# IntuitionMachines/volta

Measured on AMD Instinct MI355X. Metric: image-text pairs/sec, ctrl_vilbert_base pretrain step, higher is better.
Workload: dtype bf16

## Files before the change

include/volta_hip.h:

```cpp
#ifndef VOLTA_HIP_H
#define VOLTA_HIP_H
#include <stddef.h>
#include <stdint.h>

#ifdef __cplusplus
extern "C" {
#endif

typedef void* vk_stream_t;

int vk_version(void);
const char* vk_device_arch(void);
const char* vk_last_error(void);

typedef struct vk_dropout {
    const uint64_t* seed;
    uint32_t site;
    uint32_t threshold;
    float scale;
} vk_dropout;

int vk_set_seed(uint64_t* seed_dev, uint64_t seed, vk_stream_t s);

int vk_cast_f32_bf16(const float* src, void* dst, int64_t n, vk_stream_t s);
// ... 242 lines not shown
    const float* target;
    const int64_t* labels;
    const float* conf;
    const int32_t* pos;
    const int32_t* count;
    const int32_t* neg_index;
    float* lse;
    float* aux;
    float* loss_sum;
    float weight;
    int32_t V, ld, max_rows, kind, n_neg;
} vk_vis_loss_args;
int vk_vis_loss_fwd(const vk_vis_loss_args* a, vk_stream_t s);
int vk_vis_loss_bwd(const vk_vis_loss_args* a, void* dlogits, int ldd, const float* gscale, vk_stream_t s);
int vk_nce_negatives(vk_dropout rng, int B, int R, int32_t* out, vk_stream_t s);

enum { VK_TASK_BCE_SCALED = 0, VK_TASK_BCE_MEAN = 1, VK_TASK_BCE_REGIONS = 2, VK_TASK_CE_OPTIONS = 3 };
typedef struct vk_task_loss_args {
    const float* logits;
    const void* target;
    const int64_t* mask;
    void* work;
    float* out;
    int32_t* row_argmax;
    int32_t kind, groups, n, ld;
} vk_task_loss_args;
int64_t vk_task_loss_work_bytes(int groups);
int vk_task_loss_fwd(const vk_task_loss_args* a, vk_stream_t s);
int vk_task_loss_bwd(const vk_task_loss_args* a, const float* gscale, void* dlogits, vk_stream_t s);

int vk_mask_prep(const int64_t* mask, float* out, int n, vk_stream_t s);

#define VK_CHUNK_SKIP 255
int vk_grad_norm_workspace_floats(void);
int vk_grad_norm_clip(const float* g, int64_t n, float pre_scale, float max_norm, float* partial, float* out, vk_stream_t s);
int vk_grad_norm_clip_masked(const float* g, int64_t n, const uint8_t* chunk_class, float pre_scale, float max_norm, float* partial, float* out, vk_stream_t s);
int vk_grad_sqnorm_chunks(const float* g, int64_t chunk0, int64_t nchunks, const uint8_t* chunk_class, float* sums, vk_stream_t s);
int vk_grad_norm_from_chunks(float* sums, int64_t total_chunks, float pre_scale, float max_norm, float* out, vk_stream_t s);
typedef struct vk_adamw_args {
    float* p;
    const float* g;
    float* m;
    float* v;
    void* shadow;
    const uint8_t* chunk_class;
    const float* clip;
    int64_t n;
    float cls_lr_mult[8];
    float cls_wd[8];
    float lr, beta1, beta2, eps, step_mult, grad_scale;
} vk_adamw_args;
int vk_adamw_step(const vk_adamw_args* a, vk_stream_t s);
int vk_adamw_step_on(const vk_adamw_args* a, int ncus, vk_stream_t s);
typedef struct vk_adamw_tensor {
    float* p;
    const float* g;
    float* m;
    float* v;
    int64_t numel;
    int32_t cls;
    int32_t reserved_;
} vk_adamw_tensor;
int vk_adamw_step_list(const vk_adamw_args* a, const vk_adamw_tensor* list, int n, int64_t max_numel, vk_stream_t s);
int vk_grad_sqnorm_list(const vk_adamw_tensor* list, int n, int64_t max_numel, float* work, float* sums, vk_stream_t s);
int vk_grad_sqnorm_list_work_floats(void);
#define VK_RADAM_CLASSES 64
// ... 7 lines not shown
    const float* clip;
    int64_t n;
    float cls_decay[VK_RADAM_CLASSES];
    float cls_step[VK_RADAM_CLASSES];
    int32_t cls_rect[VK_RADAM_CLASSES];
    float beta1, beta2;
    float one_minus_beta1, one_minus_beta2;
    float eps, grad_scale;
} vk_radam_args;
int vk_radam_step(const vk_radam_args* a, vk_stream_t s);
int vk_radam_step_list(const vk_radam_args* a, const vk_adamw_tensor* list, int n, int64_t max_numel, vk_stream_t s);
int vk_axpy_f32(float* y, const float* x, float alpha, int64_t n, vk_stream_t s);
int vk_sum_slabs_f32(float* dst, const float* src, int64_t slab_stride, int nslabs, int64_t n, vk_stream_t s);
int vk_sum_slabs_bf16(void* dst, const float* src, int64_t slab_stride, int nslabs, int64_t n, const int32_t* dyn_rows, int row_len, vk_stream_t s);
int vk_memset_async(void* p, int value, int64_t bytes, vk_stream_t s);
int vk_hold_cus(int nwg, int usec, int whole_cu, vk_stream_t s);
int vk_gate_wait(const uint64_t* flag, const uint64_t* stamp, int timeout_us, int32_t* err, vk_stream_t s);
int vk_bump_u64(uint64_t* word, vk_stream_t s);
int vk_store_u64(uint64_t* word, uint64_t value, vk_stream_t s);
int vk_gate_value(const uint64_t* flag, uint64_t want, int timeout_us, int32_t* err, vk_stream_t s);
int vk_comm_standin(const void* src, void* dst, int64_t bytes, int nwg, int min_usec, uint64_t* stamps, vk_stream_t s);
int vk_gemm_reserve_cus(int n);
#define VK_TAIL_MAX_JOBS 16
typedef struct vk_tail_job {
    float* dst;
    float* dst2;
    const float* src;
    const float* src2;
    int64_t stride;
    int64_t n;
    int32_t kind, count;
    int32_t accumulate;
    int32_t block_start;
} vk_tail_job;
int vk_side_tail(const vk_tail_job* jobs, int njobs, vk_stream_t s);

int vk_mul_bf16(const void* a, const void* b, void* out, int64_t n, const int32_t* dyn_rows, int row_len, vk_stream_t s);

enum {
    VK_OP_GEMM = 1,
    VK_OP_LN_FWD, VK_OP_LN_BWD,
    VK_OP_ATTN_FWD,
    VK_OP_ATTN_BWD,
    VK_OP_EMBED_FWD, VK_OP_EMBED_BWD, VK_OP_XENT_FWD,
    VK_OP_XENT_BWD,
    VK_OP_KL_FWD, VK_OP_KL_BWD,
    VK_OP_GENERIC,
    VK_OP_SIDE_BEGIN, VK_OP_SIDE_END, VK_OP_WAIT_SIDE, VK_OP_JOIN,
    VK_OP_LN_FINALIZE,
    VK_OP_GEMM_FP8,
    VK_OP_GEMM_CHAIN
};
enum {
    VK_FN_CAST = 1, VK_FN_MEMSET, VK_FN_LOC_FWD, VK_FN_LOC_BWD, VK_FN_ADD_DROPOUT, VK_FN_COLSUM, VK_FN_SELECT,
    VK_FN_GATHER, VK_FN_SCATTER_ADD, VK_FN_LOSS_FINAL, VK_FN_POOL_FWD, VK_FN_POOL_BWD, VK_FN_MASK_PREP, VK_FN_MUL,
    VK_FN_VLBERT_PREP, VK_FN_VLBERT_MASKGRAD, VK_FN_ROWGROUP_SUM, VK_FN_RELU_BWD, VK_FN_COPY, VK_FN_SUM_SLABS, VK_FN_SUM_SLABS_BF16,
    VK_FN_SIDE_TAIL,
    VK_FN_QUANT_ROWS,
    VK_FN_CAST_FP8,
    VK_FN_VIS_LOSS_FWD,
    VK_FN_VIS_LOSS_BWD,
    VK_FN_NCE_NEG,
    VK_FN_TEXT_END_ROWS,
    VK_FN_VLBERT_OBJ_IDS,
    VK_FN_VLBERT_POSITIONS,
    VK_FN_HOLD,
// ... 129 lines not shown
```

volta_amd/_lib.py:

```python
import ctypes as C
import os

import torch

_HERE = os.path.dirname(os.path.abspath(__file__))
LIB_PATH = os.path.join(_HERE, "libvolta_hip_%s.so" % os.environ["VK_LIB"] if os.environ.get("VK_LIB") else "libvolta_hip.so")
GEMM_PERSISTENT, GEMM_ONE_TILE_PER_WG, GEMM_SOFT_START = 0x1000, 0x2000, 0x4000


class VoltaHipError(RuntimeError):
    pass


if not os.path.exists(LIB_PATH):
    raise ImportError(
        "volta_amd: %s not found. The HIP kernels are the product; there is no fallback path. "
        "Build with `make -C volta_amd/csrc` (hipcc --offload-arch=gfx950)." % LIB_PATH)

lib = C.CDLL(LIB_PATH)

c_p = C.c_void_p
i32 = C.c_int32
CHUNK_SKIP = 255


class Dropout(C.Structure):
    _fields_ = [("seed", c_p), ("site", C.c_uint32), ("threshold", C.c_uint32), ("scale", C.c_float)]


def dropout_cfg(seed_ptr, site, p):
    if p <= 0.0 or not seed_ptr:
        return Dropout(None, 0, 0, 1.0)
    return Dropout(seed_ptr, site, min(int(p * 4294967296.0), 0xFFFFFFFF), 1.0 / (1.0 - p))


def rng_cfg(seed_ptr, site):
    return Dropout(seed_ptr, site, 0, 1.0)


class GemmProblem(C.Structure):
    _fields_ = [("A", c_p), ("B", c_p), ("C", c_p), ("C2", c_p), ("bias", c_p), ("R", c_p), ("bias_grad", c_p),
                ("dyn", c_p), ("M", i32), ("N", i32), ("K", i32), ("lda", i32), ("ldb", i32), ("ldc", i32),
                ("ldr", i32), ("n_store", i32), ("ws", c_p), ("cnt", c_p), ("part", i32), ("nparts", i32),
                ("sig", c_p), ("dep", c_p), ("err", c_p), ("dep_need", i32), ("reserved_", i32), ("retire_flag", c_p), ("retire_stamp", c_p)]


class GemmFp8Problem(C.Structure):
    _fields_ = [("p", GemmProblem), ("scale_a", c_p), ("scale_b", c_p), ("c8", c_p), ("c8_mul", C.c_float), ("ldc8", i32)]


GEMM_FP8_MAX_GROUP = 4


class DropRows(C.Structure):
    _fields_ = [("site", C.c_uint32), ("div", i32), ("mul", i32), ("off", i32)]

# ... 85 lines not shown


class GradSeedArgs(C.Structure):
    _fields_ = [("src", c_p), ("stride_b", C.c_int64), ("stride_l", C.c_int64), ("dst", c_p), ("y", c_p), ("B", i32), ("L", i32), ("H", i32),
                ("row0", i32), ("ld", i32), ("ldy", i32), ("accumulate", i32), ("reserved_", i32)]


PAIR_MAX_SEGS = 8


class PairGatherArgs(C.Structure):
    _fields_ = [("src", c_p * PAIR_MAX_SEGS), ("dst", c_p * PAIR_MAX_SEGS), ("bytes", C.c_int64 * PAIR_MAX_SEGS), ("side", i32 * PAIR_MAX_SEGS),
                ("cap_idx", c_p), ("img_idx", c_p), ("n_items", C.c_int64 * 2), ("nseg", i32), ("npairs", i32), ("c0", i32), ("nc", i32),
                ("i0", i32), ("ni", i32)]


TASK_MAX_SEGS, TASK_ROWS = 2, 4
TASK_TARGET_NONE, TASK_TARGET_SCATTER, TASK_TARGET_IOU = range(3)


class TaskBatchArgs(C.Structure):
    _fields_ = [(n, c_p) for n in ("feat", "boxes", "n", "wh", "mean", "segs", "mask_count", "features", "spatials", "image_mask", "target", "csr",
                                   "labels", "scores", "ref_box")] + \
               [(n, i32) for n in ("S", "Rcap", "F", "N", "R", "B", "num_locs", "add_global", "target_kind", "num_labels")]


class TaskImage(C.Structure):
    _fields_ = [("feat_b64", c_p), ("feat_len", C.c_size_t), ("boxes_b64", c_p), ("boxes_len", C.c_size_t), ("feat", c_p), ("boxes", c_p),
                ("rows", i32), ("F", i32)]


class TailJob(C.Structure):
    _fields_ = [("dst", c_p), ("dst2", c_p), ("src", c_p), ("src2", c_p), ("stride", C.c_int64), ("n", C.c_int64), ("kind", i32), ("count", i32),
                ("accumulate", i32), ("block_start", i32)]


TAIL_MAX_JOBS = 16


class GenericArgs(C.Structure):
    _fields_ = [("fn", i32), ("p", c_p * 6), ("n", C.c_int64 * 6), ("f", C.c_float * 2), ("drop", Dropout)]


class Op(C.Structure):
    _fields_ = [("kind", i32), ("i0", i32), ("i1", i32), ("i2", i32), ("a", c_p), ("b", c_p), ("c", c_p)]


(OP_GEMM, OP_LN_FWD, OP_LN_BWD, OP_ATTN_FWD, OP_ATTN_BWD, OP_EMBED_FWD, OP_EMBED_BWD, OP_XENT_FWD, OP_XENT_BWD,
 OP_KL_FWD, OP_KL_BWD, OP_GENERIC, OP_SIDE_BEGIN, OP_SIDE_END, OP_WAIT_SIDE, OP_JOIN, OP_LN_FINALIZE, OP_GEMM_FP8, OP_GEMM_CHAIN) = range(1, 20)
(FN_CAST, FN_MEMSET, FN_LOC_FWD, FN_LOC_BWD, FN_ADD_DROPOUT, FN_COLSUM, FN_SELECT, FN_GATHER, FN_SCATTER_ADD,
 FN_LOSS_FINAL, FN_POOL_FWD, FN_POOL_BWD, FN_MASK_PREP, FN_MUL, FN_VLBERT_PREP, FN_VLBERT_MASKGRAD, FN_ROWGROUP_SUM,
 FN_RELU_BWD, FN_COPY, FN_SUM_SLABS, FN_SUM_SLABS_BF16, FN_SIDE_TAIL, FN_QUANT_ROWS, FN_CAST_FP8, FN_VIS_LOSS_FWD, FN_VIS_LOSS_BWD,
 FN_NCE_NEG, FN_TEXT_END_ROWS, FN_VLBERT_OBJ_IDS, FN_VLBERT_POSITIONS, FN_HOLD, FN_GATE, FN_BUMP, FN_GRAD_SEED) = range(1, 35)


class AttnArgs(C.Structure):
    _fields_ = [("q", c_p * 2), ("k", c_p * 2), ("v", c_p * 2), ("ld", i32 * 2), ("L", i32 * 2), ("mask", c_p * 2),
                ("ctx", c_p * 2), ("ldo", i32 * 2), ("lse", c_p * 2), ("B", i32), ("nh", i32), ("gate", (i32 * 2) * 2),
                ("drop", (Dropout * 2) * 2), ("scale", C.c_float), ("dh", i32), ("probs", (c_p * 2) * 2)]


class AttnBwdArgs(C.Structure):
    _fields_ = [("dctx", c_p * 2), ("dq", c_p * 2), ("dk", c_p * 2), ("dv", c_p * 2), ("ldg", i32 * 2)]


NT, NN, TN = 0, 1, 2
EPI_BF16, EPI_GELU, EPI_MULR, EPI_ADDR, EPI_F32, EPI_RELU, EPI_F32_ACC = range(7)
# ... 143 lines not shown
```

volta_amd/csrc/optim.hip:

```cpp
#include "common.h"
#include "../../include/volta_hip.h"
#include "util.h"

namespace vk {

constexpr int NORM_BLOCKS = 1024;

__global__ __launch_bounds__(256) void sqnorm_partial_kernel(const float* g, size_t n4, float* partial, const uint8_t* chunk_class) {
    __shared__ float sh[4];
    float s = 0.f;
    for (size_t i = (size_t)blockIdx.x * 256 + threadIdx.x; i < n4; i += (size_t)gridDim.x * 256) {
        if (chunk_class && chunk_class[i >> 8] == VK_CHUNK_SKIP) continue;
        const f32x4 v = *(const f32x4*)(g + i * 4);
        s += v[0] * v[0] + v[1] * v[1] + v[2] * v[2] + v[3] * v[3];
    }
    s = wave_sum(s);
    if ((threadIdx.x & 63) == 0) sh[threadIdx.x >> 6] = s;
    __syncthreads();
    if (threadIdx.x == 0) partial[blockIdx.x] = sh[0] + sh[1] + sh[2] + sh[3];
}
__global__ __launch_bounds__(256) void sqnorm_final_kernel(const float* partial, int nblk, float pre_scale, float max_norm, float* out) {
    __shared__ double sh[4];
    double s = 0.0;
    for (int i = threadIdx.x; i < nblk; i += 256) s += (double)partial[i];
    for (int o = 32; o > 0; o >>= 1) s += __shfl_xor(s, o, 64);
    if ((threadIdx.x & 63) == 0) sh[threadIdx.x >> 6] = s;
    __syncthreads();
    if (threadIdx.x == 0) {
        const float norm = (float)sqrt(sh[0] + sh[1] + sh[2] + sh[3]) * pre_scale;
        out[0] = norm;
        float coef = 1.f;
        if (max_norm > 0.f) { coef = max_norm / (norm + 1e-6f); if (coef > 1.f) coef = 1.f; }
        out[1] = coef;
    }
}

__global__ __launch_bounds__(256) void sqnorm_chunks_kernel(const float* g, size_t chunk0, size_t nchunks, const uint8_t* chunk_class, float* sums) {
    const size_t c = (size_t)blockIdx.x * 4 + (threadIdx.x >> 6);
    if (c >= nchunks) return;
    const size_t chunk = chunk0 + c;
    const int lane = threadIdx.x & 63;
    float s = 0.f;
    if (!(chunk_class && chunk_class[chunk] == VK_CHUNK_SKIP)) {
        const float* p = g + chunk * 1024;
#pragma unroll
        for (int k = 0; k < 4; ++k) {
            const f32x4 v = __builtin_nontemporal_load((const f32x4*)(p + (k * 64 + lane) * 4));
            s += v[0] * v[0] + v[1] * v[1] + v[2] * v[2] + v[3] * v[3];
        }
    }
    s = wave_sum(s);
    if (lane == 0) sums[chunk] = s;
}
constexpr int SQ_GROUPS = 128;
__global__ __launch_bounds__(256) void sqnorm_groups_kernel(const float* sums, size_t n, double* group) {
    __shared__ double sh[4];
    const size_t per = (n + SQ_GROUPS - 1) / SQ_GROUPS, lo = (size_t)blockIdx.x * per, hi = lo + per < n ? lo + per : n;
    double s = 0.0;
    for (size_t i = lo + threadIdx.x; i < hi; i += 256) s += (double)sums[i];
    for (int o = 32; o > 0; o >>= 1) s += __shfl_xor(s, o, 64);
    if ((threadIdx.x & 63) == 0) sh[threadIdx.x >> 6] = s;
    __syncthreads();
    if (threadIdx.x == 0) group[blockIdx.x] = (sh[0] + sh[1]) + (sh[2] + sh[3]);
}
__global__ __launch_bounds__(64) void sqnorm_from_groups_kernel(const double* group, float pre_scale, float max_norm, float* out) {
    double s = group[threadIdx.x] + group[threadIdx.x + 64];
    for (int o = 32; o > 0; o >>= 1) s += __shfl_xor(s, o, 64);
    if (threadIdx.x == 0) {
        const float norm = (float)sqrt(s) * pre_scale;
        out[0] = norm;
        float coef = 1.f;
        if (max_norm > 0.f) { coef = max_norm / (norm + 1e-6f); if (coef > 1.f) coef = 1.f; }
        out[1] = coef;
    }
}

__device__ __forceinline__ void adamw_element(float& p, float& m, float& v, float g, float gs, float b1, float b2, float eps, float step, float lr_wd) {
#pragma clang fp contract(off)
    const float gr = g * gs;
    m = __builtin_fmaf(b1, m, (1.f - b1) * gr);
    v = __builtin_fmaf(b2, v, ((1.f - b2) * gr) * gr);
    p = __builtin_fmaf(-step, m / (sqrtf(v) + eps), p);
    if (lr_wd > 0.f) p = __builtin_fmaf(-lr_wd, p, p);
}
// ... 142 lines not shown
        float a = 0.f;
        for (int s = 0; s < nslabs; ++s) a += src[(size_t)s * stride + i];
        dst[i] = a;
    }
}

__global__ __launch_bounds__(256) void sum_slabs_bf16_kernel(uint16_t* dst, const float* src, size_t stride, int nslabs, size_t n, const int32_t* dyn_rows, int row_len) {
    if (dyn_rows) { const size_t lim = (size_t)(*dyn_rows) * row_len; if (lim < n) n = lim; }
    const size_t n4 = n >> 2;
    for (size_t i = (size_t)blockIdx.x * 256 + threadIdx.x; i < n4; i += (size_t)gridDim.x * 256) {
        f32x4 a = *(const f32x4*)(src + i * 4);
        for (int s = 1; s < nslabs; ++s) {
            const f32x4 b = *(const f32x4*)(src + (size_t)s * stride + i * 4);
#pragma unroll
            for (int r = 0; r < 4; ++r) a[r] += b[r];
        }
        *(u32x2*)(dst + i * 4) = u32x2{pack2bf(a[0], a[1]), pack2bf(a[2], a[3])};
    }
}

struct TailJobs { vk_tail_job j[VK_TAIL_MAX_JOBS]; int32_t njobs; };

__global__ __launch_bounds__(256) void side_tail_kernel(const TailJobs t) {
    __shared__ float red[16][17];
    int ji = 0;
#pragma unroll
    for (int i = 1; i < VK_TAIL_MAX_JOBS; ++i)
        if (i < t.njobs && (int)blockIdx.x >= t.j[i].block_start) ji = i;
    const vk_tail_job& J = t.j[ji];
    const int blk = (int)blockIdx.x - J.block_start;
    if (J.kind == 0) {
        const size_t n4 = (size_t)J.n >> 2;
        const size_t i = (size_t)blk * 256 + threadIdx.x;
        if (i < n4) {
            f32x4 a = __builtin_nontemporal_load((const f32x4*)(J.src + i * 4));
            for (int s = 1; s < J.count; ++s) {
                const f32x4 b = __builtin_nontemporal_load((const f32x4*)(J.src + (size_t)s * J.stride + i * 4));
#pragma unroll
                for (int r = 0; r < 4; ++r) a[r] += b[r];
            }
            __builtin_nontemporal_store(a, (f32x4*)(J.dst + i * 4));
        }
        if (blk == 0 && threadIdx.x < (J.n & 3)) {
            const size_t k = n4 * 4 + threadIdx.x;
            float a = 0.f;
            for (int s = 0; s < J.count; ++s) a += J.src[(size_t)s * J.stride + k];
            J.dst[k] = a;
        }
    } else {
        const int H = (int)J.n, tx = threadIdx.x & 15, ty = threadIdx.x >> 4;
        const int i = blk * 16 + tx;
        float s = 0.f;
        if (i < 2 * H) {
            for (int b = ty; b < J.count; b += 16) s += J.src[(size_t)b * 2 * H + i];
            if (J.src2)
                for (int b = ty; b < (int)J.stride; b += 16) s += J.src2[(size_t)b * 2 * H + i];
        }
        red[ty][tx] = s;
        __syncthreads();
        if (ty == 0 && i < 2 * H) {
#pragma unroll
            for (int k = 1; k < 16; ++k) s += red[k][tx];
            float* o = i < H ? J.dst + i : J.dst2 + (i - H);
            *o = J.accumulate ? *o + s : s;
        }
    }
}

}

using namespace vk;

extern "C" int vk_side_tail(const vk_tail_job* jobs, int njobs, vk_stream_t s) {
    if (njobs <= 0) return 0;
    if (njobs > VK_TAIL_MAX_JOBS) return set_error("vk_side_tail: %d jobs (max %d)", njobs, VK_TAIL_MAX_JOBS);
    TailJobs t;
    t.njobs = njobs;
    int total = 0;
    for (int i = 0; i < njobs; ++i) {
        t.j[i] = jobs[i];
        vk_tail_job& J = t.j[i];
        int nb;
        if (J.kind == 0) {
            if ((J.stride & 3) || ((uintptr_t)J.dst & 15) || ((uintptr_t)J.src & 15)) return set_error("vk_side_tail: slab job %d needs 16-byte alignment", i);
            nb = (int)((J.n / 4 + 255) / 256);
            if (nb < 1) nb = 1;
        } else if (J.kind == 1) {
            nb = (int)((2 * J.n + 15) / 16);
        } else return set_error("vk_side_tail: unknown job kind %d", J.kind);
        if (J.n <= 0 || J.count <= 0) nb = 0;
        J.block_start = total;
        total += nb;
    }
    if (total == 0) return 0;
    hipLaunchKernelGGL(side_tail_kernel, dim3((unsigned)total), dim3(256), 0, (hipStream_t)s, t);
    return check_launch("vk_side_tail");
}

extern "C" int vk_sum_slabs_bf16(void* dst, const float* src, int64_t slab_stride, int nslabs, int64_t n, const int32_t* dyn_rows, int row_len, vk_stream_t s) {
    if (n <= 0 || nslabs <= 0) return 0;
    if ((slab_stride & 3) || (n & 3) || (row_len & 3)) return set_error("vk_sum_slabs_bf16: lengths must be multiples of 4");
    if (((uintptr_t)src & 15) || ((uintptr_t)dst & 7)) return set_error("vk_sum_slabs_bf16: src needs 16-byte, dst 8-byte alignment");
    int64_t blocks = (n / 4 + 255) / 256;
    if (blocks > 2048) blocks = 2048;
    hipLaunchKernelGGL(sum_slabs_bf16_kernel, dim3((unsigned)blocks), dim3(256), 0, (hipStream_t)s, (uint16_t*)dst, src, (size_t)slab_stride, nslabs, (size_t)n, dyn_rows, row_len);
    return check_launch("vk_sum_slabs_bf16");
}

extern "C" int vk_sum_slabs_f32(float* dst, const float* src, int64_t slab_stride, int nslabs, int64_t n, vk_stream_t s) {
    if (n <= 0 || nslabs <= 0) return 0;
    if ((slab_stride & 3) || ((uintptr_t)dst & 15) || ((uintptr_t)src & 15)) return set_error("vk_sum_slabs_f32: 16-byte alignment required");
    int64_t blocks = (n / 4 + 255) / 256;
    if (blocks > 2048) blocks = 2048;
    if (blocks < 1) blocks = 1;
    hipLaunchKernelGGL(sum_slabs_kernel, dim3((unsigned)blocks), dim3(256), 0, (hipStream_t)s, dst, src, (size_t)slab_stride, nslabs, (size_t)n);
    return check_launch("vk_sum_slabs_f32");
}

extern "C" int vk_grad_norm_workspace_floats(void) { return NORM_BLOCKS; }

extern "C" int vk_grad_norm_clip_masked(const float* g, int64_t n, const uint8_t* chunk_class, float pre_scale, float max_norm, float* partial, float* out, vk_stream_t s) {
// ... 83 lines not shown
```

volta_amd/engine.py:

```python
import ctypes as C
import math
import os

import torch

from . import _lib as L
from ._lib import check, ptr
from .modules import sublayer_schedule

CHUNK = 1024
VIS_TARGET_WIDTH = {"0": 1601, "1": 2048, "2": 2048, "3": 1600, "4": 400, "5": 2048, "6": 1601}
NO_DECAY = ("bias", "LayerNorm.bias", "LayerNorm.weight")


def _round_up(x, m):
    return (x + m - 1) // m * m


class ParamArena:

    def __init__(self, model, device, prefix=""):
        named = [(prefix + n, p) for n, p in model.named_parameters()]
        byname = dict(named)
        slots, seen = [], set()
# ... 13 lines not shown
        self.offset, self.shape = {}, {}
        classes = []
        off = 0
        for group in slots:
            start = off
            for g in group:
                self.offset[g] = off
                self.shape[g] = tuple(byname[g].shape)
                off += byname[g].numel()
            off = _round_up(off, CHUNK)
            nd = any(k in group[0] for k in NO_DECAY)
            assert all(any(k in g for k in NO_DECAY) == nd for g in group)
            classes += [1 if nd else 0] * ((off - start) // CHUNK)
        self.total = off
        self.device = device
        self.master = torch.zeros(self.total, dtype=torch.float32, device=device)
        self.shadow = torch.zeros(self.total, dtype=torch.bfloat16, device=device)
        self.grad = torch.zeros(self.total, dtype=torch.float32, device=device)
        self.chunk_class = torch.tensor(classes, dtype=torch.uint8, device=device)
        self.names = [n for n, _ in named]
        self.params = byname
        with torch.no_grad():
            for name, p in named:
                v = self.view(name)
                v.copy_(p.data.to(device=device, dtype=torch.float32))
                p.data = v
                p.grad = None
        self.shadow_version = -1
        self.weights_epoch = 0
        self.fp8_sites = {}
        self.fp8_epoch = -1
        self._plist = self._gviews = None
        self.opt_pending = None

    def view(self, name, which="master"):
        buf = getattr(self, which)
        o = self.offset[name]
        n = 1
        for d in self.shape[name]:
            n *= d
        return buf[o:o + n].view(self.shape[name])

    def param_list(self):
        if self._plist is None or len(self._plist) != len(self.params):
            self._plist = list(self.params.items())
        return self._plist

    def grad_views(self):
        if self._gviews is None or len(self._gviews) != len(self.params):
            self._gviews = [self.view(n, "grad") for n in self.params]
        return self._gviews

    def span(self, names, which, shape):
        buf = getattr(self, which)
        o = self.offset[names[0]]
        n = 1
        for d in shape:
            n *= d
        for a, b in zip(names[:-1], names[1:]):
            assert self.offset[b] == self.offset[a] + int(torch.tensor(self.shape[a]).prod())
        return buf[o:o + n].view(shape)

    def intact(self):
        return all(p.data_ptr() == self.master.data_ptr() + 4 * self.offset[n] for n, p in self.params.items())

    def param_version(self):
        return sum(p._version for p in self.params.values()) + self.master._version

    def refresh_shadow(self, force=False):
        v = self.param_version()
        if force or self.shadow_version != v:
            self.sync_optimizer()
            check(L.lib.vk_cast_f32_bf16(ptr(self.master), ptr(self.shadow), self.total, L.stream_ptr()))
            self.shadow_version = v
            self.weights_epoch += 1

    def mark_shadow_fresh(self):
        self.shadow_version = self.param_version()
        self.weights_epoch += 1

    def fp8_weight(self, w):
        key = w.data_ptr()
        if key not in self.fp8_sites:
            N, K = w.shape
            Kp = _round_up(K, 128)
            self.fp8_sites[key] = (w, torch.zeros(N, Kp, dtype=torch.uint8, device=self.device), torch.ones(N, dtype=torch.float32, device=self.device))
            self.fp8_epoch = -1
        return self.fp8_sites[key][1:]

    def refresh_fp8(self):
        if self.fp8_epoch == self.weights_epoch:
            return
        for w, q, sc in self.fp8_sites.values():
            N, K = w.shape
# ... 105 lines not shown
        if self.wide and fp8:
            raise NotImplementedError("the fp8 projection path covers the single-width (ctrl_*) geometry")
        if self.wide and cfg.image_embeddings != "vilbert":
            raise NotImplementedError("different stream widths are built for the ViLBERT embeddings (config/vilbert_base.json)")
        if cfg.hidden_act != "gelu" or cfg.v_hidden_act != "gelu":
            raise NotImplementedError("engine supports gelu activations (every reference config)")
        if cfg.fusion_method not in ("mul", "sum", "text", "vl-bert_vqa", "none"):
            raise ValueError("Invalid fusion method: %s" % cfg.fusion_method)
        self.unused_params = set()
        if T + Rv > 512:
            raise NotImplementedError("more than 512 keys per query row (%d text + %d vision rows)" % (T, Rv))
        self.H, self.I, self.nh = H, cfg.intermediate_size, cfg.num_attention_heads
        self.st = [Stream(T, B, H), Stream(Rv, B, Hv)]
        self.R = Rv - (1 if cfg.add_global_imgfeat is not None else 0)
        self.bufs = {}
        self.keep = []
        self.fwd, self.bwd = Plan(), Plan()
        self.bwd_groups = []
        self.site = 0
        self.seed = torch.zeros(1, dtype=torch.int64, device=dev)
        self.inputs = {}
        self.taps = {}
        self.grad_seeds = {}
        self.losses = None
        self.nce_site = None
        self.task_loss_bufs = None
        self._aside = ""
        self._split_cur = {}
        self._soft_zero_b_listed = False
        self._n_ln_partial = 0
        self._deferred_ln = []
        self._n_gate, self._gate_flag = 0, None
        self._slab_cursor = 0
        self._fwd_segments = {}
        self._build()

    def buf(self, name, shape, dtype=torch.bfloat16, zero=False):
        assert name not in self.bufs, name
        t = (torch.zeros if zero else torch.empty)(shape, dtype=dtype, device=self.dev)
        self.bufs[name] = t
        return t

    def embed_ws(self, eb, tag):
        n = L.lib.vk_embed_bwd_workspace_bytes(eb.M, eb.H, eb.V, eb.P, int(bool(eb.pos_ids) and bool(eb.dpos)))
        eb.work = _addr(self.tmp("embed_ws_" + tag, (max(n, 1),), torch.uint8))
        return eb

    def tmp(self, name, shape, dtype=torch.bfloat16):
        name += self._aside
        if name not in self.bufs:
            self.bufs[name] = torch.empty(shape, dtype=dtype, device=self.dev)
        t = self.bufs[name]
        assert tuple(t.shape) == tuple(shape) and t.dtype == dtype, (name, t.shape, shape)
        return t

    def drop(self, p):
        site = self.site
        self.site += 1
        return L.dropout_cfg(self.seed.data_ptr(), site, p if self.train else 0.0)

    def k(self, obj):
        self.keep.append(obj)
        return obj

    def patch(self, name, struct, field, index=None):
        self.inputs.setdefault(name, []).append((struct, field, index))
# ... 216 lines not shown
        self.sublayer_ids = [n for n, _ in sched]
        backbone = self.heads == "backbone"
        v_level0 = []
        for k, (n, typ) in enumerate(sched):
            self.sub_k = k
            self.fwd_sub_start.append(len(self.fwd.ops))
            if emb_image_aside and k == k_vis:
                f.append((L.OP_WAIT_SIDE, 15, 0, 0, None, None, None))
            ops = self._attn_sublayer(n) if typ == "attn" else self._ffn_sublayer(n)
            if k + 2 < self.n_sub:
                ops.insert(0, (L.OP_WAIT_SIDE, (k + 2) % 8, 0, 0, None, None, None))
            if backbone and k + 1 < self.n_sub:
                head = []
                for m, tag in ((0, "t"), (1, "v")):
                    op = self._seed_op("%s%d" % (tag, n), self._dx(m, self.level[m] % 2), self.B, self.st[m].L, self.st[m].H, accumulate=1)
                    (v_level0 if (m == 1 and emb_image_aside and self.level[1] == 0) else head).append(op)
                ops[0:0] = head
            if emb_image_aside and k == k_vis:
                ops = ops + v_level0 + emb_image_bwd
            bwd_stages.append(ops)
            self.taps["t%d" % n], self.taps["v%d" % n] = self.x[0], self.x[1]
        self.fwd_heads_start = len(self.fwd.ops)
        head_bwd = self._heads() if self.heads == "pretrain" else self._heads_tasks()
        self.bwd.ops = list(self.bwd_pro) + list(head_bwd)
        self.bwd_marks = [len(self.bwd.ops)]
        for ops in reversed(bwd_stages):
            self.bwd.ops += ops
            self.bwd_marks.append(len(self.bwd.ops))
        self.bwd.ops.append((L.OP_JOIN, 0, 0, 0, None, None, None))
        prefixes = [["bert.t_pooler.", "bert.v_pooler.", "cls.", "clfs_dict."]] + [pf for pf in reversed(self.stage_prefix)]
        self.param_ready_stage = {}
        for name in self.arena.params:
            self.param_ready_stage[name] = max(i for i, pf in enumerate(prefixes) if any(name.startswith(q) for q in pf))
        self.fwd.freeze()
        self.bwd.freeze()

    def _build_score(self):
        cfg, B, T, Rv = self.cfg, self.B, self.T, self.Rv
        f = self.fwd.ops
        text_subs, vision_subs, per_modality = self.split
        kinds = dict(sublayer_schedule(cfg))
        self.x, self.x8, self.level, self.bwd_pro = [None, None], [None, None], [0, 0], []
        self.masks = [self.buf("mask_t", (B, T), torch.float32), self.buf("mask_v", (B, Rv), torch.float32)]
        kind = cfg.image_embeddings

        def mask_prep(m, src=None):
            g = self.generic(L.FN_MASK_PREP, p=(src, self.masks[m]), n=(B * self.st[m].L,))
            if src is None:
                self.patch(("attention_mask", "image_attention_mask")[m], g, "p", 0)
            f.append((L.OP_GENERIC, 0, 0, 0, g, None, None))

        def sublayers(ns):
            for n in ns:
                self._attn_sublayer(n) if kinds[n] == "attn" else self._ffn_sublayer(n)

        if self.part in ("text", "image"):
            m = 0 if self.part == "text" else 1
            subs = text_subs if m == 0 else vision_subs
            if not per_modality:
                raise ValueError("image_embeddings=%r mixes the modalities in its embedding: there is no per-modality prefix" % kind)
            if subs:
                mask_prep(m)
            if m == 0:
                self._emb_text("bert.embeddings.")
            elif kind == "uniter":
                self._emb_image_uniter("bert.embeddings.")
# ... 649 lines not shown
            du[m] = self.tmp("du%d_%d%s" % (m, par, wtag), (self.st[m].M, Im[m]))
        self._ln_pair(b, L.OP_LN_BWD, lnb)
        d1 = [self.prob(dd[m], self.W(names[m]["down"] + ".weight"), du[m], self.st[m].M, Im[m], Hm[m], Hm[m], Im[m], Im[m], R=gp[m], ldr=Im[m]) for m in ms]
        d2 = [self.prob(du[m], self.W(names[m]["up"] + ".weight"), dxn[m], self.st[m].M, Hm[m], Im[m], Im[m], Hm[m], Hm[m], R=dz[m], ldr=Hm[m]) for m in ms]
        chained = self.chain == "all" and not self.fp8 and self._soft_pair_ok([(self.st[m].M, Im[m], Hm[m]) for m in ms])
        if chained:
            for m, p1, p2 in zip(ms, d1, d2):
                p1.sig, p1.err = self.soft_counters(self.st[m].M // 256, backward=True)
                p2.dep, p2.err, p2.dep_need = p1.sig, p1.err, Im[m] // 256
            self.gemm_chain(b, L.NN, L.EPI_MULR, d1, L.EPI_ADDR, d2)
        else:
            self.gemm(b, L.NN, L.EPI_MULR, d1)
        gate_mode, self.side_gate = self.side_gate, self.side_gate and not chained
        self._wgrad(b, ms, shared, [lambda m: (dd[m], h[m], self.G(names[m]["down"] + ".weight"), self.G(names[m]["down"] + ".bias"), Hm[m], Im[m], Hm[m], Im[m]),
                                    lambda m: (du[m], x_in[m], self.G(names[m]["up"] + ".weight"), self.G(names[m]["up"] + ".bias"), Im[m], Hm[m], Im[m], Hm[m])])
        self.side_gate = gate_mode
        if not chained:
            self.gemm(b, L.NN, L.EPI_ADDR, self.retire_on(d2))
        return b

    def _wgrad(self, b, ms, shared, specs):
        jobs = []
        for spec in specs:
            per_w = {}
            for m in ms:
                dY, X, gW, gB, Mo, No, lda, ldb = spec(m)
                key = gW.data_ptr()
                per_w.setdefault(key, (gW, gB, Mo, No, []))[4].append((dY, X, self.st[m].M, lda, ldb))
            jobs += list(per_w.values())
        chunk_rows = 5120.0
        tiles = lambda cr: sum(-(-Mo // 256) * -(-No // 256) * sum(max(1, int(round(rows / cr))) for _, _, rows, _, _ in srcs) for _, _, Mo, No, srcs in jobs)
        while chunk_rows > 1280 and tiles(chunk_rows) < 130:
            chunk_rows /= 2
        probs, reduces = [], []
        for gW, gB, Mo, No, srcs in jobs:
            chunks = []
            for dY, X, rows, lda, ldb in srcs:
                ns = max(1, int(round(rows / chunk_rows)))
                step = -(-rows // ns)
                step = -(-step // 64) * 64
                r0 = 0
                while r0 < rows:
                    chunks.append((dY[r0:], X[r0:], min(step, rows - r0), lda, ldb))
                    r0 += step
            if len(chunks) == 1:
                dY, X, rows, lda, ldb = chunks[0]
                probs.append(self.prob(dY, X, gW, Mo, No, rows, lda, ldb, No, bias_grad=gB))
                continue
            stride = _round_up(Mo * No + Mo, 4)
            slab = self._slab(len(chunks) * stride)
            for i, (dY, X, rows, lda, ldb) in enumerate(chunks):
                base = slab[i * stride:]
                probs.append(self.prob(dY, X, base, Mo, No, rows, lda, ldb, No, bias_grad=base[Mo * No:]))
            reduces.append((gW, slab, stride, len(chunks), Mo * No))
            reduces.append((gB, slab[Mo * No:], stride, len(chunks), Mo))
        assert len(probs) <= 32, "too many wgrad problems in one group"
        gate = self._gate_words() if self.side_gate else None
        b.append((L.OP_SIDE_BEGIN, 1 if gate is not None else 0, 0, 0, None, None, None))
        if gate is not None:
            self._n_gate += 1
            assert self._n_gate < gate.numel()
            flag = gate.data_ptr() + 8 * self._n_gate
            b.append((L.OP_GENERIC, 0, 0, 0, self.generic(L.FN_GATE, p=(flag, gate.data_ptr(), self.bufs["gate_err"]), n=(1000000,)), None, None))
            self._gate_flag = (flag, gate.data_ptr())
        if self.side_delay_us > 0:
            b.append((L.OP_GENERIC, 0, 0, 0, self.generic(L.FN_HOLD, n=(1, self.side_delay_us, 0)), None, None))
        self.gemm(b, L.TN, L.EPI_F32, probs)
        jobs = [L.TailJob(_addr(dst), None, _addr(src), None, stride, n, 0, ns, 0, 0) for dst, src, stride, ns, n in reduces]
        by_dst = {}
        for a in self._deferred_ln:
            by_dst.setdefault(a.dgamma, []).append(a)
        for group in by_dst.values():
            assert len(group) <= 2 and not (group[0].accumulate & 1) and all(g.accumulate & 1 for g in group[1:]), "unexpected LayerNorm sharing"
            a, b2 = group[0], (group[1] if len(group) > 1 else None)
            jobs.append(L.TailJob(a.dgamma, a.dbeta, a.partial, b2.partial if b2 else None, L.lib.vk_ln_bwd_partial_rows(b2.M) if b2 else 0, a.H, 1,
                                  L.lib.vk_ln_bwd_partial_rows(a.M), 0, 0))
        self._deferred_ln = []
        for i in range(0, len(jobs), L.TAIL_MAX_JOBS):
            chunk = jobs[i:i + L.TAIL_MAX_JOBS]
            arr = self.k((L.TailJob * len(chunk))(*chunk))
            b.append((L.OP_GENERIC, 0, 0, 0, self.generic(L.FN_SIDE_TAIL, p=(arr,), n=(len(chunk),)), None, None))
        b.append((L.OP_SIDE_END, self.sub_k % 8, 0, 0, None, None, None))
        self._slab_cursor = 0

    def _gate_words(self):
        if "gate_words" not in self.bufs:
            self.bufs["gate_words"] = torch.zeros(128, dtype=torch.int64, device=self.dev)
            self.bufs["gate_words"][1:] = -1
            self.bufs["gate_err"] = torch.zeros(1, dtype=torch.int32, device=self.dev)
            g = self.bufs["gate_words"]
            self.bwd_pro.append((L.OP_GENERIC, 0, 0, 0, self.generic(L.FN_BUMP, p=(g,)), None, None))
            self.bwd_pro.append((L.OP_SIDE_BEGIN, 0, 0, 0, None, None, None))
            self.bwd_pro.append((L.OP_SIDE_END, 13, 0, 0, None, None, None))
        return self.bufs["gate_words"]

    def retire_on(self, probs):
        gf = self._gate_flag
        if gf is not None:
            probs[0].retire_flag, probs[0].retire_stamp = gf
            self._gate_flag = None
        return probs

    def _slab(self, n):
        cap = 48 * 3072 * 768
        ws = self.tmp("wgrad_slabs", (cap,), torch.float32)
        cur = _round_up(self._slab_cursor, 4)
        assert cur + n <= cap, "wgrad slab workspace too small"
        self._slab_cursor = cur + n
        return ws[cur:cur + n]

    def _heads(self):
        cfg, B, H, T, Rv, R = self.cfg, self.B, self.H, self.T, self.Rv, self.R
        Hv = self.st[1].H
        f = self.fwd.ops
        st_t, st_v = self.st
        fm = cfg.fusion_method
# ... 442 lines not shown
```

volta_amd/modeling.py:

```python
import logging
import os

import torch
from torch import nn

from . import modules as M
from .config import BertConfig

logger = logging.getLogger(__name__)


class ArenaParameters:

    __slots__ = ("vk_model", "started", "_it")

    def __init__(self, model, it):
        self.vk_model, self.started, self._it = model, False, it

    def __iter__(self):
        return self

    def __next__(self):
        self.started = True
        return next(self._it)
# ... 253 lines not shown
        anchor = next((p for p in self.parameters() if p.requires_grad), None) if node is not None and torch.is_grad_enabled() else None
        if anchor is not None:
            return node.apply(self, anchor, *args)
        with torch.no_grad():
            return eager(*args)

    def _backward_begin(self, eng, absent=()):
        arena = eng.arena
        from .optimization import flush_clip
        flush_clip(arena)
        skip = self._torch_param_prefixes
        unused = eng.unused_params
        pairs = [((n, p), g) for (n, p), g in zip(arena.param_list(), arena.grad_views())
                 if p.requires_grad and not (skip and n.startswith(skip)) and n not in unused and n not in absent]
        params, gviews = [x[0] for x in pairs], [x[1] for x in pairs]
        n_have = sum(p.grad is not None for _, p in params)
        accumulate = n_have == len(params)
        if n_have and not accumulate:
            raise RuntimeError("volta_amd: some parameters carry a .grad and some do not; zero_grad() all of them")
        old = None
        if accumulate:
            if not all(p.grad is g or p.grad.data_ptr() == g.data_ptr() for (_, p), g in zip(params, gviews)):
                raise RuntimeError("volta_amd: .grad tensors were replaced by foreign tensors; call zero_grad(set_to_none=True)")
            old = arena.grad.clone()
        return params, gviews, accumulate, old

    def _backward_run(self, eng, state):
        params, gviews, accumulate, old = state
        arena = eng.arena
        skip = self._torch_param_prefixes
        if skip:
            keep = [(g, g.clone()) for (n, _), g in zip(arena.param_list(), arena.grad_views()) if n.startswith(skip)] if accumulate else []
        ddp = self._ddp
        if ddp is not None:
            ddp.run_backward(eng)
        else:
            eng.bwd.run()
        if accumulate:
            from . import _lib as L
            L.check(L.lib.vk_axpy_f32(L.ptr(arena.grad), L.ptr(old), 1.0, arena.total, L.stream_ptr()))
            if skip:
                for g, saved in keep:
                    g.copy_(saved)
        else:
            for (_, p), g in zip(params, gviews):
                p.grad = g

    def _encode_labels(self, B, T, R, dev):
        return {}

    def encode(self, input_ids, image_feat, image_loc, token_type_ids=None, attention_mask=None, image_attention_mask=None,
               output_all_encoded_layers=False, output_all_attention_masks=False):
        B, T = input_ids.shape
        labels = self._encode_labels(B, T, image_feat.shape[1] - self.add_global_imgfeat, next(self.parameters()).device)
        tensors, B, T, Rv = self._prep_inputs(input_ids, image_feat, image_loc, token_type_ids, attention_mask, image_attention_mask, **labels)
        self._run_step(None, self._engine_forward, tensors, None, output_all_attention_masks and self.config.visualization)
        eng = self._last[0]
        attn_maps = _attention_maps(self.config, eng, output_all_attention_masks)
        H, Hv = self.config.hidden_size, self.config.v_hidden_size
        pt, pv = eng.taps["pooled_t"], eng.taps["pooled_v"]
        if output_all_encoded_layers:
            seq_t = [eng.taps["t%d" % n].view(B, T, H).float() for n in eng.sublayer_ids]
            seq_v = [eng.taps["v%d" % n].view(B, Rv, Hv).float() for n in eng.sublayer_ids]
        else:
            seq_t, seq_v = eng.taps["seq_t"].view(B, T, H).float(), eng.taps["seq_v"].view(B, Rv, Hv).float()
        return seq_t, seq_v, None if pt is None else pt.float(), None if pv is None else pv.float(), attn_maps


class _BackboneStep(torch.autograd.Function):

# ... 424 lines not shown
```

volta_amd/optimization.py:

```python
import ctypes as C
import math
import os

import numpy as np
import torch
import weakref

from torch.optim import Optimizer
from torch.optim.lr_scheduler import LambdaLR

from . import _lib as L


def _split_params(params, labels=None):
    labels = labels or ["parameter %d" % i for i in range(len(params))]
    owners, foreign = {}, []
    for p, lab in zip(params, labels):
        o = getattr(p, "_vk_owner", None)
        if o is not None:
            owners.setdefault(id(o), (o, lab))
        else:
            foreign.append((p, lab))
    if len(owners) > 1:
        (_, a), (_, b) = list(owners.values())[:2]
# ... 707 lines not shown
        given = {p.data_ptr() for p in params}
    flush_clip(arena)
    plist, gviews = arena.param_list(), arena.grad_views()
    have = []
    for (n, p), g in zip(plist, gviews):
        if not whole and p.data_ptr() not in given:
            continue
        if p.grad is None:
            continue
        if not (p.grad is g or p.grad.data_ptr() == g.data_ptr()):
            raise RuntimeError("clip_grad_norm_: the gradient of %s is not attached to the engine's arena (run backward first)" % n)
        have.append(n)
    if not have and not any(p.grad is not None for p in foreign):
        raise RuntimeError("clip_grad_norm_: gradients are not attached to the engine's arena (run backward first)")
    flive = [p for p in foreign if p.grad is not None]
    if flive and _red_mode(model) == "zero1":
        raise NotImplementedError("clip_grad_norm_: data-parallel mode 'zero1' with parameters outside the model's arena")
    mask = None
    if len(have) != len(plist):
        cache = arena.__dict__.setdefault("_clip_masks", {})
        key = tuple(have)
        if key not in cache:
            if len(cache) > 16:
                cache.clear()
            _check_shared_chunks(arena, set(have), "part of the norm")
            cc = torch.full((arena.total // 1024,), L.CHUNK_SKIP, dtype=torch.uint8)
            for n in have:
                c0, c1 = _chunks_of(arena, n)
                cc[c0:c1] = 0
            cache[key] = cc.to(arena.device)
        mask = cache[key]
    nchunks = arena.total // 1024
    npad = nchunks + (nchunks & 1)
    if not hasattr(arena, "norm_chunks"):
        arena.norm_chunks = torch.zeros(npad + 256, device=arena.device)
    sums = arena.norm_chunks[:npad]
    if flive:
        nf = len(flive)
        npad = nchunks + nf + ((nchunks + nf) & 1)
        buf = arena.__dict__.get("norm_slots")
        if buf is None or buf.numel() < npad + 256:
            buf = arena.__dict__["norm_slots"] = torch.zeros(npad + 256, device=arena.device)
        sums = buf[:npad]
        sums[nchunks + nf:].zero_()
        ents = [(p, p.grad, None, None, 0) for p in flive]
        for p in flive:
            if p.grad.dtype != torch.float32 or not p.grad.is_contiguous() or p.grad.device != arena.device:
                raise RuntimeError("clip_grad_norm_: the gradient of a tensor outside the arena must be a contiguous float32 tensor on %s" % arena.device)
        flist, fmax = _tensor_list(ents, arena.device)
        work = torch.empty(nf * L.lib.vk_grad_sqnorm_list_work_floats(), device=arena.device)
        L.check(L.lib.vk_grad_sqnorm_list(L.ptr(flist), nf, fmax, L.ptr(work), L.ptr(sums[nchunks:]), L.stream_ptr()))
    out = torch.empty(2, device=arena.device)
    ddp = getattr(model, "_ddp", None)
    red = getattr(ddp, "reducer", None)
    if red is not None and red.mode == "zero1" and (red.sharded or red.replicated):
        sums.zero_()
        mine = [(lo + red.rank * s, lo + (red.rank + 1) * s) for lo, hi, s in red.sharded] + (list(red.replicated) if red.rank == 0 else [])
        for lo, hi in mine:
            L.check(L.lib.vk_grad_sqnorm_chunks(L.ptr(arena.grad), lo // 1024, (hi - lo) // 1024, L.ptr(mask), L.ptr(sums), L.stream_ptr()))
        torch.distributed.all_reduce(sums, group=red.pg)
    else:
        L.check(L.lib.vk_grad_sqnorm_chunks(L.ptr(arena.grad), 0, nchunks, L.ptr(mask), L.ptr(sums), L.stream_ptr()))
    L.check(L.lib.vk_grad_norm_from_chunks(L.ptr(sums), npad, pre_scale, float(max_norm), L.ptr(out), L.stream_ptr()))
    names = frozenset(have + [("foreign", id(p)) for p in flive])
    if defer_to_optimizer is None:
        opt = getattr(arena, "_vk_adamw", None)
        opt = opt() if opt is not None else None
        defer_to_optimizer = opt is not None and opt._fused is not None and opt._fused["arena"] is arena and opt._grad_names() == names
    arena.pending_clip = (out, names, [p.grad for p in flive]) if flive else (out, names)
    if not defer_to_optimizer:
        flush_clip(arena)
    return out[0]


def _red_mode(model):
    red = getattr(getattr(model, "_ddp", None), "reducer", None)
    return red.mode if red is not None and (red.sharded or red.replicated) else None


def _clip_foreign_only(params, max_norm, pre_scale):
    live = [p for p in params if p.grad is not None]
    if not live:
        raise RuntimeError("clip_grad_norm_: no parameter carries a gradient")
    dev = live[0].device
    nf = len(live)
    npad = nf + (nf & 1)
    sums = torch.zeros(npad + 256, device=dev)
    flist, fmax = _tensor_list([(p, p.grad, None, None, 0) for p in live], dev)
    work = torch.empty(nf * L.lib.vk_grad_sqnorm_list_work_floats(), device=dev)
    L.check(L.lib.vk_grad_sqnorm_list(L.ptr(flist), nf, fmax, L.ptr(work), L.ptr(sums), L.stream_ptr()))
    out = torch.empty(2, device=dev)
    L.check(L.lib.vk_grad_norm_from_chunks(L.ptr(sums), npad, pre_scale, float(max_norm), L.ptr(out), L.stream_ptr()))
    for p in live:
        p.grad.mul_(out[1])
    return out[0]
```

Baseline: 15320.

## Compute gradient-norm chunk sums early inside backward side-tail reductions

Weight-gradient slab reductions in the side stream now also write the per-1024-element squared-norm chunk sums while the reduced values are still in registers, and a new chunk-sum job kind covers directly produced gradients. Chunks already summed are tagged DONE in the clip mask, so the later norm pass skips rereading them from memory. This trades a second full read of much of the gradient arena for extra work in the side tail, plus bookkeeping (version checks, alignment requirements, cached masks) that only applies in the non-DDP, non-accumulating path. Summation order is kept fixed so the norm value matches the standalone pass.

```diff
diff --git a/include/volta_hip.h b/include/volta_hip.h
--- a/include/volta_hip.h
+++ b/include/volta_hip.h
@@ -298,6 +298,7 @@
 int vk_mask_prep(const int64_t* mask, float* out, int n, vk_stream_t s);
 
 #define VK_CHUNK_SKIP 255
+#define VK_CHUNK_DONE 254
 int vk_grad_norm_workspace_floats(void);
 int vk_grad_norm_clip(const float* g, int64_t n, float pre_scale, float max_norm, float* partial, float* out, vk_stream_t s);
 int vk_grad_norm_clip_masked(const float* g, int64_t n, const uint8_t* chunk_class, float pre_scale, float max_norm, float* partial, float* out, vk_stream_t s);
@@ -371,6 +372,8 @@
     int32_t kind, count;
     int32_t accumulate;
     int32_t block_start;
+    float* sums;
+    int64_t chunk;
 } vk_tail_job;
 int vk_side_tail(const vk_tail_job* jobs, int njobs, vk_stream_t s);
 
diff --git a/volta_amd/_lib.py b/volta_amd/_lib.py
--- a/volta_amd/_lib.py
+++ b/volta_amd/_lib.py
@@ -22,6 +22,7 @@
 c_p = C.c_void_p
 i32 = C.c_int32
 CHUNK_SKIP = 255
+CHUNK_DONE = 254
 
 
 class Dropout(C.Structure):
@@ -173,7 +174,7 @@
 
 class TailJob(C.Structure):
     _fields_ = [("dst", c_p), ("dst2", c_p), ("src", c_p), ("src2", c_p), ("stride", C.c_int64), ("n", C.c_int64), ("kind", i32), ("count", i32),
-                ("accumulate", i32), ("block_start", i32)]
+                ("accumulate", i32), ("block_start", i32), ("sums", c_p), ("chunk", C.c_int64)]
 
 
 TAIL_MAX_JOBS = 16
diff --git a/volta_amd/csrc/optim.hip b/volta_amd/csrc/optim.hip
--- a/volta_amd/csrc/optim.hip
+++ b/volta_amd/csrc/optim.hip
@@ -35,21 +35,29 @@
     }
 }
 
+__device__ __forceinline__ float sq_piece(const f32x4 v) {
+#pragma clang fp contract(off)
+    return __builtin_fmaf(v[3], v[3], __builtin_fmaf(v[2], v[2], __builtin_fmaf(v[0], v[0], v[1] * v[1])));
+}
+__device__ __forceinline__ float sq_chunk(float q0, float q1, float q2, float q3) {
+#pragma clang fp contract(off)
+    return wave_sum(((q0 + q1) + q2) + q3);
+}
+__device__ __forceinline__ float sq_chunk_load(const float* p, int lane) {
+    float q[4];
+#pragma unroll
+    for (int k = 0; k < 4; ++k) q[k] = sq_piece(__builtin_nontemporal_load((const f32x4*)(p + (k * 64 + lane) * 4)));
+    return sq_chunk(q[0], q[1], q[2], q[3]);
+}
+
 __global__ __launch_bounds__(256) void sqnorm_chunks_kernel(const float* g, size_t chunk0, size_t nchunks, const uint8_t* chunk_class, float* sums) {
     const size_t c = (size_t)blockIdx.x * 4 + (threadIdx.x >> 6);
     if (c >= nchunks) return;
     const size_t chunk = chunk0 + c;
     const int lane = threadIdx.x & 63;
-    float s = 0.f;
-    if (!(chunk_class && chunk_class[chunk] == VK_CHUNK_SKIP)) {
-        const float* p = g + chunk * 1024;
-#pragma unroll
-        for (int k = 0; k < 4; ++k) {
-            const f32x4 v = __builtin_nontemporal_load((const f32x4*)(p + (k * 64 + lane) * 4));
-            s += v[0] * v[0] + v[1] * v[1] + v[2] * v[2] + v[3] * v[3];
-        }
-    }
-    s = wave_sum(s);
+    const int cls = chunk_class ? chunk_class[chunk] : 0;
+    if (cls == VK_CHUNK_DONE) return;
+    const float s = cls == VK_CHUNK_SKIP ? 0.f : sq_chunk_load(g + chunk * 1024, lane);
     if (lane == 0) sums[chunk] = s;
 }
 constexpr int SQ_GROUPS = 128;
@@ -258,8 +266,9 @@
     if (J.kind == 0) {
         const size_t n4 = (size_t)J.n >> 2;
         const size_t i = (size_t)blk * 256 + threadIdx.x;
+        f32x4 a = {0.f, 0.f, 0.f, 0.f};
         if (i < n4) {
-            f32x4 a = __builtin_nontemporal_load((const f32x4*)(J.src + i * 4));
+            a = __builtin_nontemporal_load((const f32x4*)(J.src + i * 4));
             for (int s = 1; s < J.count; ++s) {
                 const f32x4 b = __builtin_nontemporal_load((const f32x4*)(J.src + (size_t)s * J.stride + i * 4));
 #pragma unroll
@@ -272,6 +281,22 @@
             float a = 0.f;
             for (int s = 0; s < J.count; ++s) a += J.src[(size_t)s * J.stride + k];
             J.dst[k] = a;
+        }
+        if (J.sums && ((size_t)blk + 1) * 1024 <= (size_t)J.n) {
+            float* q = &red[0][0];
+            q[threadIdx.x] = sq_piece(a);
+            __syncthreads();
+            if (threadIdx.x < 64) {
+                const float s = sq_chunk(q[threadIdx.x], q[64 + threadIdx.x], q[128 + threadIdx.x], q[192 + threadIdx.x]);
+                if (threadIdx.x == 0) J.sums[J.chunk + blk] = s;
+            }
+        }
+    } else if (J.kind == 2) {
+        const size_t c = (size_t)blk * 4 + (threadIdx.x >> 6);
+        if (c < ((size_t)J.n >> 10)) {
+            const int lane = threadIdx.x & 63;
+            const float s = sq_chunk_load(J.src + c * 1024, lane);
+            if (lane == 0) J.sums[J.chunk + c] = s;
         }
     } else {
         const int H = (int)J.n, tx = threadIdx.x & 15, ty = threadIdx.x >> 4;
@@ -311,8 +336,13 @@
             if ((J.stride & 3) || ((uintptr_t)J.dst & 15) || ((uintptr_t)J.src & 15)) return set_error("vk_side_tail: slab job %d needs 16-byte alignment", i);
             nb = (int)((J.n / 4 + 255) / 256);
             if (nb < 1) nb = 1;
+            if ((uintptr_t)J.dst & 4095) J.sums = nullptr;
+            if (J.sums && J.chunk < 0) return set_error("vk_side_tail: slab job %d has a negative chunk index", i);
         } else if (J.kind == 1) {
             nb = (int)((2 * J.n + 15) / 16);
+        } else if (J.kind == 2) {
+            if (!J.sums || !J.src || J.chunk < 0 || (J.n & 1023) || ((uintptr_t)J.src & 15)) return set_error("vk_side_tail: chunk-sum job %d needs sums, whole 1024-element chunks and 16-byte alignment", i);
+            nb = (int)((J.n / 1024 + 3) / 4);
         } else return set_error("vk_side_tail: unknown job kind %d", J.kind);
         if (J.n <= 0 || J.count <= 0) nb = 0;
         J.block_start = total;
diff --git a/volta_amd/engine.py b/volta_amd/engine.py
--- a/volta_amd/engine.py
+++ b/volta_amd/engine.py
@@ -69,6 +69,7 @@
         self.fp8_epoch = -1
         self._plist = self._gviews = None
         self.opt_pending = None
+        self.early_sums = None
 
     def view(self, name, which="master"):
         buf = getattr(self, which)
@@ -97,6 +98,12 @@
         for a, b in zip(names[:-1], names[1:]):
             assert self.offset[b] == self.offset[a] + int(torch.tensor(self.shape[a]).prod())
         return buf[o:o + n].view(shape)
+
+    def norm_sums(self):
+        if not hasattr(self, "norm_chunks"):
+            nchunks = self.total // CHUNK
+            self.norm_chunks = torch.zeros(nchunks + (nchunks & 1) + 256, device=self.device)
+        return self.norm_chunks
 
     def intact(self):
         return all(p.data_ptr() == self.master.data_ptr() + 4 * self.offset[n] for n, p in self.params.items())
@@ -268,6 +275,8 @@
         self._deferred_ln = []
         self._n_gate, self._gate_flag = 0, None
         self._slab_cursor = 0
+        self._early = [] if arena.grad.data_ptr() % (4 * CHUNK) == 0 else None
+        self.early_done = None
         self._fwd_segments = {}
         self._build()
 
@@ -550,6 +559,12 @@
         self.param_ready_stage = {}
         for name in self.arena.params:
             self.param_ready_stage[name] = max(i for i, pf in enumerate(prefixes) if any(name.startswith(q) for q in pf))
+        if self._early:
+            done = torch.zeros(self.arena.total // CHUNK, dtype=torch.uint8)
+            for c0, c1, _ in self._early:
+                assert not done[c0:c1].any(), "a gradient chunk has two producers"
+                done[c0:c1] = 1
+            self.early_done = done.to(self.dev)
         self.fwd.freeze()
         self.bwd.freeze()
 
@@ -1265,7 +1280,7 @@
         tiles = lambda cr: sum(-(-Mo // 256) * -(-No // 256) * sum(max(1, int(round(rows / cr))) for _, _, rows, _, _ in srcs) for _, _, Mo, No, srcs in jobs)
         while chunk_rows > 1280 and tiles(chunk_rows) < 130:
             chunk_rows /= 2
-        probs, reduces = [], []
+        probs, reduces, direct = [], [], []
         for gW, gB, Mo, No, srcs in jobs:
             chunks = []
             for dY, X, rows, lda, ldb in srcs:
@@ -1279,6 +1294,7 @@
             if len(chunks) == 1:
                 dY, X, rows, lda, ldb = chunks[0]
                 probs.append(self.prob(dY, X, gW, Mo, No, rows, lda, ldb, No, bias_grad=gB))
+                direct += [(gW, Mo * No), (gB, Mo)]
                 continue
             stride = _round_up(Mo * No + Mo, 4)
             slab = self._slab(len(chunks) * stride)
@@ -1299,7 +1315,20 @@
         if self.side_delay_us > 0:
             b.append((L.OP_GENERIC, 0, 0, 0, self.generic(L.FN_HOLD, n=(1, self.side_delay_us, 0)), None, None))
         self.gemm(b, L.TN, L.EPI_F32, probs)
-        jobs = [L.TailJob(_addr(dst), None, _addr(src), None, stride, n, 0, ns, 0, 0) for dst, src, stride, ns, n in reduces]
+        jobs = []
+        for dst, src, stride, ns, n in reduces:
+            c0, c1 = self._grad_chunks(dst, n)
+            if self._early is not None and self._grad_offset(dst) == c0 * CHUNK and c1 > c0:
+                self._early.append((c0, c1, 0))
+                jobs.append(L.TailJob(_addr(dst), None, _addr(src), None, stride, n, 0, ns, 0, 0, self.arena.norm_sums().data_ptr(), c0))
+            else:
+                jobs.append(L.TailJob(_addr(dst), None, _addr(src), None, stride, n, 0, ns, 0, 0))
+        for dst, n in direct if self._early is not None else ():
+            c0, c1 = self._grad_chunks(dst, n)
+            if c1 > c0:
+                self._early.append((c0, c1, 2))
+                jobs.append(L.TailJob(None, None, self.arena.grad.data_ptr() + 4 * CHUNK * c0, None, 0, (c1 - c0) * CHUNK, 2, 1, 0, 0,
+                                      self.arena.norm_sums().data_ptr(), c0))
         by_dst = {}
         for a in self._deferred_ln:
             by_dst.setdefault(a.dgamma, []).append(a)
@@ -1315,6 +1344,15 @@
             b.append((L.OP_GENERIC, 0, 0, 0, self.generic(L.FN_SIDE_TAIL, p=(arr,), n=(len(chunk),)), None, None))
         b.append((L.OP_SIDE_END, self.sub_k % 8, 0, 0, None, None, None))
         self._slab_cursor = 0
+
+    def _grad_offset(self, t):
+        off = (t.data_ptr() - self.arena.grad.data_ptr()) // 4
+        assert 0 <= off < self.arena.total, "not a view of the gradient arena"
+        return off
+
+    def _grad_chunks(self, t, n):
+        off = self._grad_offset(t)
+        return -(-off // CHUNK), (off + n) // CHUNK
 
     def _gate_words(self):
         if "gate_words" not in self.bufs:
diff --git a/volta_amd/modeling.py b/volta_amd/modeling.py
--- a/volta_amd/modeling.py
+++ b/volta_amd/modeling.py
@@ -309,10 +309,13 @@
         if skip:
             keep = [(g, g.clone()) for (n, _), g in zip(arena.param_list(), arena.grad_views()) if n.startswith(skip)] if accumulate else []
         ddp = self._ddp
+        arena.early_sums = None
         if ddp is not None:
             ddp.run_backward(eng)
         else:
             eng.bwd.run()
+            if not accumulate and eng.early_done is not None:
+                arena.early_sums = (eng.early_done, tuple(n for n, _ in params), arena.grad._version)
         if accumulate:
             from . import _lib as L
             L.check(L.lib.vk_axpy_f32(L.ptr(arena.grad), L.ptr(old), 1.0, arena.total, L.stream_ptr()))
diff --git a/volta_amd/optimization.py b/volta_amd/optimization.py
--- a/volta_amd/optimization.py
+++ b/volta_amd/optimization.py
@@ -763,9 +763,7 @@
         mask = cache[key]
     nchunks = arena.total // 1024
     npad = nchunks + (nchunks & 1)
-    if not hasattr(arena, "norm_chunks"):
-        arena.norm_chunks = torch.zeros(npad + 256, device=arena.device)
-    sums = arena.norm_chunks[:npad]
+    sums = arena.norm_sums()[:npad]
     if flive:
         nf = len(flive)
         npad = nchunks + nf + ((nchunks + nf) & 1)
@@ -791,6 +789,8 @@
             L.check(L.lib.vk_grad_sqnorm_chunks(L.ptr(arena.grad), lo // 1024, (hi - lo) // 1024, L.ptr(mask), L.ptr(sums), L.stream_ptr()))
         torch.distributed.all_reduce(sums, group=red.pg)
     else:
+        if red is None and not flive:
+            mask = _early_mask(arena, have, mask)
         L.check(L.lib.vk_grad_sqnorm_chunks(L.ptr(arena.grad), 0, nchunks, L.ptr(mask), L.ptr(sums), L.stream_ptr()))
     L.check(L.lib.vk_grad_norm_from_chunks(L.ptr(sums), npad, pre_scale, float(max_norm), L.ptr(out), L.stream_ptr()))
     names = frozenset(have + [("foreign", id(p)) for p in flive])
@@ -802,6 +802,23 @@
     if not defer_to_optimizer:
         flush_clip(arena)
     return out[0]
+
+
+def _early_mask(arena, have, mask):
+    early = arena.early_sums
+    if early is None:
+        return mask
+    done, names, version = early
+    if version != arena.grad._version or len(names) != len(have) or names != tuple(have):
+        return mask
+    cache = arena.__dict__.setdefault("_early_masks", {})
+    key = (done.data_ptr(), None if mask is None else mask.data_ptr())
+    if key not in cache:
+        if len(cache) > 16:
+            cache.clear()
+        base = torch.zeros_like(done) if mask is None else mask
+        cache[key] = (torch.where(done.bool() & (base != L.CHUNK_SKIP), torch.full_like(done, L.CHUNK_DONE), base), done, mask)
+    return cache[key][0]
 
 
 def _red_mode(model):
```

Result: no change. 15400 (median of 6 runs) (+0.5%).
